# titu1994/tfdiffeq

Hardware: NVIDIA H100
Metric: accepted_rk_steps_x_state_elements_per_s (higher is better)
Workload: dtype f64

## Files before the change

### tfdiffeq_b200/csrc/b2ode_fused.cu

```cuda

#include "b2ode_dev.cuh"
#include "b2ode_rhs.cuh"
#include "b2ode_pay16.cuh"
#include <stdlib.h>
#include <mutex>

#ifdef B2ODE_FUSED_TRACE
constexpr int kTraceAttempts = 64, kTracePhases = 16;
__device__ unsigned long long g_fused_trace[2 * kTraceAttempts * kTracePhases];
#define FTRACE_DEP(att, ph, dep)                                                                                 \
    do {                                                                                                         \
        if ((unsigned)(dep) != 0x7ffffff3u && (threadIdx.x == 0 || threadIdx.x == blockDim.x - 32)  &&            \
            (blockIdx.x == 0 || blockIdx.x == gridDim.x - 1) && (att) >= 8 && (att) < 8 + kTraceAttempts)        \
            g_fused_trace[((blockIdx.x == 0 ? 0 : 1) * kTraceAttempts + ((att)-8)) * kTracePhases + (ph)] = clock64(); \
    } while (0)
#define FTRACE(att, ph) FTRACE_DEP(att, ph, 0)
extern "C" int b2ode_debug_fused_trace(unsigned long long *out) {
    B2_CUDA(cudaMemcpyFromSymbol(out, g_fused_trace, sizeof(g_fused_trace)));
    return 0;
}
#else
#define FTRACE(att, ph) do { } while (0)
#define FTRACE_DEP(att, ph, dep) do { } while (0)
#endif


struct FusedParams {
    b2ode_state *st;
    unsigned long long *part2;
    unsigned *ctr;
    const void *y0;
    void *out;
    unsigned *progress;
    int *host_mark;
    long long n_traj;
    int ncw;
    int have_first_step;
    double t_start, first_step;
    double time_sign;
    double rhs[8];
    const void *rhs_data;
    double beta[B2ODE_MAXK][B2ODE_MAXK];
    double c_sol[B2ODE_MAXK], c_error[B2ODE_MAXK], c_mid[B2ODE_MAXK];
    int fsal;
    double rtol0, atol0;
    CtrlParams c;
    CommParams comm;
};

__device__ __forceinline__ unsigned long long umax64(unsigned long long a, unsigned long long b) { return a > b ? a : b; }

template <int MODE>
__device__ __forceinline__ Pay pay_identity() {
    Pay r;
    r.a = 0.0;
    r.b = 0ull;
    r.flag = 0u;
    return r;
}

template <int MODE>
__device__ __forceinline__ Pay pay_combine(const Pay &x, const Pay &y) {
    Pay r;
    r.a = x.a + y.a;
    if (MODE == 0) r.b = x.b > y.b ? x.b : y.b;
    else r.b = (unsigned long long)__double_as_longlong(__longlong_as_double((long long)x.b) + __longlong_as_double((long long)y.b));
    r.flag = x.flag | y.flag;
    return r;
}

template <int MODE>
__device__ __forceinline__ Pay pay_warp_reduce(Pay x) {
#pragma unroll
    for (int o = 16; o > 0; o >>= 1) {
        Pay y;
        y.a = __shfl_xor_sync(0xffffffffu, x.a, o);
        y.b = __shfl_xor_sync(0xffffffffu, x.b, o);
        y.flag = __shfl_xor_sync(0xffffffffu, x.flag, o);
        x = pay_combine<MODE>(x, y);
    }
    return x;
}

__device__ __forceinline__ void pay_pack(const Pay &x, unsigned seq, unsigned long long (&w)[4]) {
    unsigned long long ab = (unsigned long long)__double_as_longlong(x.a);
    if (x.a != x.a) ab = 0x7ff8000000000000ull;
    ab = (ab & 0x7fffffffffffffffull) | ((unsigned long long)(x.flag & 1u) << 63);
    const unsigned long long s = (unsigned long long)seq << 32;
    w[0] = s | (ab & 0xffffffffull);
    w[1] = s | (ab >> 32);
    w[2] = s | (x.b & 0xffffffffull);
    w[3] = s | (x.b >> 32);
}

__device__ __forceinline__ Pay pay_unpack(const unsigned long long (&w)[4]) {
    const unsigned long long ab = (w[0] & 0xffffffffull) | (w[1] << 32);
    Pay r;
    r.flag = (unsigned)(ab >> 63);
    r.a = __longlong_as_double((long long)(ab & 0x7fffffffffffffffull));
    r.b = (w[2] & 0xffffffffull) | (w[3] << 32);
    return r;
}

template <bool SYS>
__device__ __forceinline__ void ll_store4(unsigned long long *dst, const unsigned long long (&w)[4]) {
    if (SYS) {
        asm volatile("st.relaxed.sys.global.v2.u64 [%0], {%1, %2};" ::"l"(dst), "l"(w[0]), "l"(w[1]) : "memory");
        asm volatile("st.relaxed.sys.global.v2.u64 [%0], {%1, %2};" ::"l"(dst + 2), "l"(w[2]), "l"(w[3]) : "memory");
    } else {
        asm volatile("st.relaxed.gpu.global.v2.u64 [%0], {%1, %2};" ::"l"(dst), "l"(w[0]), "l"(w[1]) : "memory");
        asm volatile("st.relaxed.gpu.global.v2.u64 [%0], {%1, %2};" ::"l"(dst + 2), "l"(w[2]), "l"(w[3]) : "memory");
    }
}

template <bool SYS>
__device__ __forceinline__ Pay ll_wait4(const unsigned long long *src, unsigned seq) {
    unsigned long long w[4];
    for (;;) {
        if (SYS) {
            asm volatile("ld.relaxed.sys.global.v2.u64 {%0, %1}, [%2];" : "=l"(w[0]), "=l"(w[1]) : "l"(src) : "memory");
            asm volatile("ld.relaxed.sys.global.v2.u64 {%0, %1}, [%2];" : "=l"(w[2]), "=l"(w[3]) : "l"(src + 2) : "memory");
        } else {
            asm volatile("ld.relaxed.gpu.global.v2.u64 {%0, %1}, [%2];" : "=l"(w[0]), "=l"(w[1]) : "l"(src) : "memory");
            asm volatile("ld.relaxed.gpu.global.v2.u64 {%0, %1}, [%2];" : "=l"(w[2]), "=l"(w[3]) : "l"(src + 2) : "memory");
        }
        if ((unsigned)(w[0] >> 32) == seq && (unsigned)(w[1] >> 32) == seq && (unsigned)(w[2] >> 32) == seq &&
            (unsigned)(w[3] >> 32) == seq)
            break;
    }
    return pay_unpack(w);
}

__device__ __forceinline__ void named_arrive(int id, int count) { asm volatile("bar.arrive %0, %1;" ::"r"(id), "r"(count) : "memory"); }
__device__ __forceinline__ void named_sync(int id, int count) { asm volatile("bar.sync %0, %1;" ::"r"(id), "r"(count) : "memory"); }

__device__ __forceinline__ unsigned long long opaque_zero() {
    unsigned long long c;
    asm volatile("mov.u64 %0, %%clock64;" : "=l"(c));
    return c >> 63;
}

constexpr int kGatherPerLane = 5;

struct FusedShared {
    Pay part[32];
    unsigned long long rlane[B2ODE_MAXPEERS][32][2];
    Pay tot;
    struct {
        double dt_next;
        int accept, done;
        unsigned status;
    } ctl;
};

constexpr int kBarPartials = 1, kBarDecision = 2, kBarRows = 3, kBarRowsReady = 4, kBarRemote = 5;

template <typename T, int S>
struct DenseConst {
    T cmid[S];
    T fc[5];
};

template <typename T>
__device__ __forceinline__ T fit_coef(int q) { return q == 0 ? T(-2) : q == 1 ? T(2) : q == 2 ? T(5) : q == 3 ? T(-3) : T(-4); }

template <typename T, int S>
__device__ __forceinline__ DenseConst<T, S> dense_const(const FusedParams &p, T dtc) {
    DenseConst<T, S> dc;
#pragma unroll
    for (int j = 0; j < S; ++j) dc.cmid[j] = Ar<T>::mul(dtc, (T)p.c_mid[j]);
#pragma unroll
    for (int q = 0; q < 5; ++q) dc.fc[q] = Ar<T>::mul(fit_coef<T>(q), dtc);
    return dc;
}

template <typename T, int S>
struct DenseShared {
    DenseConst<T, S> k;
    T x[3][4];
};

template <int MODE>
__device__ __forceinline__ void remote_gather(const FusedParams &p, FusedShared &sh, unsigned seq) {
    const int nranks = p.comm.nranks, lane = threadIdx.x & 31, rank = p.comm.rank;
#ifndef B2ODE_COMM_RG
#define B2ODE_COMM_RG 3
#endif
    constexpr int RG = B2ODE_COMM_RG;
    constexpr int NL = RG * kGatherPerLane;
    const unsigned long long *base = &p.comm.box[rank]->fused_part[seq & 1u][0][0][0] + (size_t)lane * 2;
    const unsigned tag = pay_tag(seq);
    for (int i0 = 0; i0 < nranks - 1; i0 += RG) {
        unsigned long long g0[NL], g1[NL];
        const unsigned long long *ptr[RG];
        unsigned mine = 0u;
#pragma unroll
        for (int r = 0; r < RG; ++r) {
            const int i = i0 + r;
            const bool ok = i < nranks - 1;
            const int src = ok ? (i < rank ? i : i + 1) : rank;
            const int G = ok ? p.comm.grid_of[src] : 0;
            ptr[r] = base + (size_t)src * (kMaxFusedBlocks * 2);
            asm volatile("" : "+l"(ptr[r]));
#pragma unroll
            for (int q = 0; q < kGatherPerLane; ++q)
                if (lane + 32 * q < G) mine |= 1u << (r * kGatherPerLane + q);
        }
        unsigned got;
        do {
            const unsigned long long z = opaque_zero();
#pragma unroll
            for (int r = 0; r < RG; ++r)
#pragma unroll
                for (int q = 0; q < kGatherPerLane; ++q)
                    asm volatile("ld.global.cg.v2.u64 {%0, %1}, [%2];"
                                 : "=l"(g0[r * kGatherPerLane + q]), "=l"(g1[r * kGatherPerLane + q])
                                 : "l"(ptr[r] + z + 64 * q)
                                 : "memory");
            got = 0u;
#pragma unroll
            for (int k = 0; k < NL; ++k) {
                got |= (pay_mismatch(g0[k], g1[k], tag) == 0u) ? (1u << k) : 0u;
            }
        } while ((got & mine) != mine);
#pragma unroll
        for (int r = 0; r < RG; ++r) {
            const int i = i0 + r;
            if (i >= nranks - 1) continue;
            const int src = i < rank ? i : i + 1;
            Pay acc = pay_identity<MODE>();
#pragma unroll
            for (int q = 0; q < kGatherPerLane; ++q)
                if ((mine >> (r * kGatherPerLane + q)) & 1u)
                    acc = pay_combine<MODE>(acc, pay_unpack16(g0[r * kGatherPerLane + q], g1[r * kGatherPerLane + q]));
            const int G = p.comm.grid_of[src];
            for (int b = lane + 32 * kGatherPerLane; b < G; b += 32) {
                const unsigned long long *sl = base + (size_t)src * (kMaxFusedBlocks * 2) + (size_t)(b - lane) * 2;
                unsigned long long a0, a1;
                do {
                    asm volatile("ld.global.cg.v2.u64 {%0, %1}, [%2];" : "=l"(a0), "=l"(a1) : "l"(sl + opaque_zero()) : "memory");
                } while (!pay_valid16(a0, a1, seq));
                acc = pay_combine<MODE>(acc, pay_unpack16(a0, a1));
            }
#ifdef B2ODE_COMM_RTOT
            acc = pay_warp_reduce<MODE>(acc);
#endif
            unsigned long long ab = (unsigned long long)__double_as_longlong(acc.a);
            if (acc.a != acc.a) ab = 0x7ff8000000000000ull;
            sh.rlane[src][lane][0] = (ab & 0x7fffffffffffffffull) | ((unsigned long long)(acc.flag & 1u) << 63);
            sh.rlane[src][lane][1] = acc.b;
        }
    }
    asm volatile("bar.arrive %0, %1;" ::"r"(kBarRemote), "r"(64) : "memory");
}

template <int MODE>
__device__ __forceinline__ Pay control_allreduce(const FusedParams &p, FusedShared &sh, int ncw, unsigned epoch, unsigned seq0,
                                                 unsigned long long hw2 = 0ull ,
                                                 int att = -1) {
    const int lane = threadIdx.x & 31;
    Pay x = (lane < ncw) ? sh.part[lane] : pay_identity<MODE>();
    x = pay_warp_reduce<MODE>(x);
    FTRACE_DEP(att, 2, __double_as_longlong(x.a));
    const int nranks = p.comm.nranks > 1 ? p.comm.nranks : 1, rank = p.comm.rank;
    const int G = (int)gridDim.x;
    const unsigned seq = seq0 + epoch, par = seq & 1u;
    unsigned long long w0, w1;
    pay_pack16(x, seq, w0, w1);
    if (nranks > 1 && epoch <= 2u && lane < nranks && lane != rank) {
        const int hw = (int)(par ? (unsigned)(hw2 >> 32) : (unsigned)hw2);
        for (int b = G + (int)blockIdx.x; b < hw && b < kMaxFusedBlocks; b += G) {
            unsigned long long *dst = &p.comm.box[lane]->fused_part[par][rank][b][0];
            asm volatile("st.relaxed.sys.global.v2.u64 [%0], {%1, %2};" ::"l"(dst), "l"(kPoisonW0), "l"(kPoisonW1) : "memory");
        }
    }
    if (nranks > 1 && lane < nranks && lane != rank) {
        unsigned long long *dst = &p.comm.box[lane]->fused_part[par][rank][blockIdx.x][0];
        asm volatile("st.relaxed.sys.global.v2.u64 [%0], {%1, %2};" ::"l"(dst), "l"(w0), "l"(w1) : "memory");
    }
    if (G > 1) {
        unsigned long long *slots = p.part2 + (size_t)par * G * 2;
        if (lane == 0) {
            asm volatile("st.relaxed.gpu.global.v2.u64 [%0], {%1, %2};" ::"l"(slots + (size_t)blockIdx.x * 2), "l"(w0), "l"(w1) : "memory");
            asm volatile("red.relaxed.gpu.global.add.u32 [%0], 1;" ::"l"(p.ctr) : "memory");
            const unsigned target = epoch * (unsigned)G;
            unsigned v;
            do {
                asm volatile("ld.relaxed.gpu.global.u32 %0, [%1];" : "=r"(v) : "l"(p.ctr) : "memory");
            } while ((int)(v - target) < 0);
        }
        __syncwarp();
        FTRACE(att, 3);
        unsigned long long g0[kGatherPerLane], g1[kGatherPerLane];
#pragma unroll
        for (int q = 0; q < kGatherPerLane; ++q) {
            const int b = lane + 32 * q;
            asm volatile("ld.global.cg.v2.u64 {%0, %1}, [%2];" : "=l"(g0[q]), "=l"(g1[q]) : "l"(slots + (size_t)(b < G ? b : 0) * 2) : "memory");
        }
        x = pay_identity<MODE>();
#pragma unroll
        for (int q = 0; q < kGatherPerLane; ++q) {
            const int b = lane + 32 * q;
            if (b < G) {
                while (!pay_valid16(g0[q], g1[q], seq))
                    asm volatile("ld.relaxed.gpu.global.v2.u64 {%0, %1}, [%2];" : "=l"(g0[q]), "=l"(g1[q]) : "l"(slots + (size_t)b * 2) : "memory");
                x = pay_combine<MODE>(x, pay_unpack16(g0[q], g1[q]));
            }
        }
        for (int b = lane + 32 * kGatherPerLane; b < G; b += 32) {
            unsigned long long a0, a1;
            do {
                asm volatile("ld.relaxed.gpu.global.v2.u64 {%0, %1}, [%2];" : "=l"(a0), "=l"(a1) : "l"(slots + (size_t)b * 2) : "memory");
            } while (!pay_valid16(a0, a1, seq));
            x = pay_combine<MODE>(x, pay_unpack16(a0, a1));
        }
    } else {
        x = (lane == 0) ? pay_unpack16(w0, w1) : pay_identity<MODE>();
    }
    if (nranks == 1) return pay_warp_reduce<MODE>(x);
#ifdef B2ODE_COMM_RTOT
    x = pay_warp_reduce<MODE>(x);
#endif
    asm volatile("bar.sync %0, %1;" ::"r"(kBarRemote), "r"(64) : "memory");
    Pay tot = pay_identity<MODE>();
    for (int q = 0; q < nranks; ++q) {
        Pay v = x;
        if (q != rank) {
            const unsigned long long a = sh.rlane[q][lane][0];
            v.flag = (unsigned)(a >> 63);
            v.a = __longlong_as_double((long long)(a & 0x7fffffffffffffffull));
            v.b = sh.rlane[q][lane][1];
        }
        tot = (q == 0) ? v : pay_combine<MODE>(tot, v);
    }
#ifdef B2ODE_COMM_RTOT
    return tot;
#else
    return pay_warp_reduce<MODE>(tot);
#endif
}

template <typename T>
__device__ __forceinline__ CtrlDecision ctrl_fast(const CtrlParams &c, double ssq, double mm, bool bad0, double dt) {
    const T tol = Ar<T>::add((T)c.atol[0], Ar<T>::mul((T)c.rtol[0], (T)mm));
    const double tol2n = (double)tol * (double)tol * (double)c.n_global[0];
    const double bound = std::is_same<T, float>::value ? tol2n * (1.0 + 5.9604644775390625e-08) : tol2n;
    CtrlDecision d;
    d.bad0 = bad0;
    d.accept = ssq <= bound;
    {
        const double lg = log2(((threadIdx.x & 31) == 0) ? ssq : tol2n);
        const double L = __shfl_sync(0xffffffffu, lg, 0) - __shfl_sync(0xffffffffu, lg, 1);
        const double df = (ssq < tol2n) ? 1.0 : c.dfactor;
        const double rf = c.safety * exp2(-0.5 * c.exponent * L);
        d.dt_next = (ssq == 0.0) ? dt * c.ifactor : dt * nan_min(c.ifactor, nan_max(df, rf));
    }
    d.m = 0.0;
    return d;
}


constexpr int fused_warps(int ntw, int tpt, int nsvc) { return (ntw + tpt - 1) / tpt + nsvc; }
constexpr int cmax(int a, int b) { return a > b ? a : b; }

template <typename T, typename RHS, int S, int MAXT>
struct FusedShape {
    static constexpr int tpt = (S == 7 && !(std::is_same<T, double>::value && RHS::D > 3)) ? 2 : 1;
    static constexpr int threads = 32 * cmax(fused_warps(MAXT / 32 - 1, tpt, 1), fused_warps(MAXT / 32 - 2, tpt, 2));
    static constexpr int min_blocks = tpt > 1 ? 1 : 0;
};

template <typename T, typename RHS, int S, int MAXT>
__global__ void __launch_bounds__(FusedShape<T, RHS, S, MAXT>::threads, FusedShape<T, RHS, S, MAXT>::min_blocks)
k_fused_adaptive(const __grid_constant__ FusedParams p) {
    constexpr int TPT = FusedShape<T, RHS, S, MAXT>::tpt;
    using A = Ar<T>;
    constexpr int D = RHS::D;
    constexpr int kMaxTraj = MAXT - 32;
    __shared__ FusedShared sh;
    __shared__ T sw[RHS::kSmem];
    __shared__ DenseShared<T, S> sdc;
    constexpr int kDenseRows = (3 * kMaxTraj * D * (int)sizeof(T) + (int)sizeof(FusedShared) + RHS::kSmem * (int)sizeof(T) +
                                (int)sizeof(DenseShared<T, S>) + 256 <= 48 * 1024) ? 3 : 2;
    __shared__ __align__(16) T s_rows[kDenseRows][kMaxTraj * D];
    const int nthreads = blockDim.x;
    const bool grouped = p.comm.nranks > 1;
    const int nsvc = grouped ? 2 : 1;
    const int pcw = (nthreads >> 5) - nsvc;
    const int ncw = p.ncw;
    const int nloc = 32 * (pcw + 1);
    const int warp = threadIdx.x >> 5, lane = threadIdx.x & 31;
    const bool is_control = warp == pcw;
    const unsigned ll_base = grouped ? (unsigned)p.comm.box[p.comm.rank]->ll_seq : 0u;
    const unsigned long long hw2 = (grouped && is_control) ? *(const volatile unsigned long long *)p.comm.box[p.comm.rank]->fused_hw : 0ull;
    if (RHS::kSmem > 1) {
        const int nw = (int)p.rhs[0] * 5 + 2;
        for (int q = threadIdx.x; q < nw && q < RHS::kSmem; q += nthreads) sw[q] = ((const T *)p.rhs_data)[q];
        __syncthreads();
    }
    const int n_out = p.c.n_out;
    const double *__restrict__ t_out = p.c.t_out;

    if (is_control) {
        unsigned epoch = 0;
        double t_cur = p.t_start, dt;
        unsigned status = 0;
        if (p.have_first_step) {
            dt = p.first_step;
        } else {
            named_sync(kBarPartials, nloc);
            Pay r = control_allreduce<1>(p, sh, ncw, ++epoch, ll_base, hw2);
            if (lane == 0) sh.tot = r;
            named_arrive(kBarDecision, nthreads);
            Partial tot;
            tot.v[0] = r.a;
            tot.v[1] = __longlong_as_double((long long)r.b);
            tot.v[2] = tot.v[3] = 0.0;
            T d1max;
            const T h0 = init_h0<T>(p.c, &tot, 1, &d1max);
            named_sync(kBarPartials, nloc);
            r = control_allreduce<1>(p, sh, ncw, ++epoch, ll_base, hw2);
            if (lane == 0) sh.tot = r;
            named_arrive(kBarDecision, nthreads);
            tot.v[0] = r.a;
            dt = (double)init_dt<T>(p.c, &tot, 1, h0, d1max);
        }
        int cur = 1;
        int done = (n_out <= 1) ? 1 : 0;
        if (!done && !(t_cur + dt > t_cur)) {
            status |= B2ODE_ST_UNDERFLOW;
            done = 1;
        }
        int late_rows = 0;
        double m_last = 0.0, t_prev = t_cur, dt_last = 0.0;
        unsigned long long n_acc = 0, n_rej = 0;
        long long nadv = 0;
        int att = 0;
        while (!done) {
            FTRACE(att, 0);
            const double t1_acc = t_cur + dt;
            int c2 = cur;
            while (c2 < n_out && __ldg(t_out + c2) <= t1_acc) ++c2;
            if (c2 > cur) {
                const T dtc = (T)dt, t0s = (T)t_cur, den = A::sub((T)t1_acc, t0s);
                if (lane < S) sdc.k.cmid[lane] = A::mul(dtc, (T)p.c_mid[lane]);
                if (lane < 5) sdc.k.fc[lane] = A::mul(fit_coef<T>(lane), dtc);
                if (lane < kDenseRows && cur + lane < c2) {
                    const T x = A::div(A::sub((T)__ldg(t_out + cur + lane), t0s), den);
                    const T x2 = A::mul(x, x), x3 = A::mul(x2, x), x4 = A::mul(x3, x);
                    sdc.x[lane][0] = x;
                    sdc.x[lane][1] = x2;
                    sdc.x[lane][2] = x3;
                    sdc.x[lane][3] = x4;
                }
                named_arrive(kBarRows, nloc);
            }
            named_sync(kBarPartials, nloc);
            if (late_rows) {
                __threadfence();
                if (lane == 0) {
                    const unsigned old = atomicAdd(p.progress, (unsigned)late_rows);
                    if (old + (unsigned)late_rows == (unsigned)(cur - 1) * gridDim.x) {
                        __threadfence_system();
                        *(volatile int *)p.host_mark = cur;
                    }
                }
                late_rows = 0;
            }
            FTRACE_DEP(att, 1, sh.part[0].flag);
            const Pay r = control_allreduce<0>(p, sh, ncw, ++epoch, ll_base, hw2, att);
            FTRACE_DEP(att, 4, __double_as_longlong(r.a));
            Partial tot;
            tot.v[0] = r.a;
            tot.v[1] = tot.v[2] = __longlong_as_double((long long)r.b);
            tot.v[3] = r.flag ? 1.0 : 0.0;
            CtrlDecision dec = ctrl_fast<T>(p.c, tot.v[0], tot.v[1], r.flag != 0u, dt);
            unsigned st_bits = status;
            if (dec.bad0) st_bits |= B2ODE_ST_NONFINITE;
            const bool adv = dec.accept && !dec.bad0;
            const double t1n = dec.accept ? t1_acc : t_cur;
            const int c_new = adv ? c2 : cur;
            const long long nadv2 = (c_new > cur) ? 0 : nadv + 1;
            int dn = (c_new >= n_out) ? 1 : 0;
            if (!dn) {
                if (nadv2 >= p.c.max_num_steps) st_bits |= B2ODE_ST_MAXSTEPS;
                if (!(t1n + dec.dt_next > t1n)) st_bits |= B2ODE_ST_UNDERFLOW;
            }
            if (st_bits) dn = 1;
            if (lane == 0) {
                sh.ctl.dt_next = dec.dt_next;
                sh.ctl.accept = dec.accept ? 1 : 0;
                sh.ctl.done = dn;
                sh.ctl.status = st_bits;
            }
            named_arrive(kBarDecision, nthreads);
            FTRACE_DEP(att, 5, __double_as_longlong(dec.dt_next));
            if (c2 > cur) named_sync(kBarRowsReady, nloc);
            if (adv && c2 > cur) {
                const long long first = (long long)blockIdx.x * (ncw * 32);
                long long nblk = p.n_traj - first;
                if (nblk > ncw * 32) nblk = ncw * 32;
                const int nel = (int)(nblk > 0 ? nblk * D : 0);
                const long long Nrow = p.n_traj * D;
                const int nrows = (c2 - cur) < kDenseRows ? (c2 - cur) : kDenseRows;
                for (int q = 0; q < nrows; ++q) {
                    T *row = (T *)p.out + (long long)(cur + q) * Nrow + first * D;
                    const T *src = s_rows[q];
                    constexpr int V = 16 / sizeof(T);
                    if ((reinterpret_cast<uintptr_t>(row) & 15u) == 0) {
                        const int nv = nel / V;
                        for (int e = lane; e < nv; e += 32)
                            reinterpret_cast<int4 *>(row)[e] = reinterpret_cast<const int4 *>(src)[e];
                        for (int e = nv * V + lane; e < nel; e += 32) row[e] = src[e];
                    } else {
                        for (int e = lane; e < nel; e += 32) row[e] = src[e];
                    }
                }
                if (p.host_mark) {
                    if (c2 - cur > kDenseRows) {
                        late_rows = c2 - cur;
                    } else {
                        __threadfence();
                        if (lane == 0) {
                            const unsigned old = atomicAdd(p.progress, (unsigned)(c2 - cur));
                            if (old + (unsigned)(c2 - cur) == (unsigned)(c2 - 1) * gridDim.x) {
                                __threadfence_system();
                                *(volatile int *)p.host_mark = c2;
                            }
                        }
                    }
                }
            }
            {
                const T tol = Ar<T>::add((T)p.c.atol[0], Ar<T>::mul((T)p.c.rtol[0], (T)tot.v[1]));
                dec.m = (double)(T)(tot.v[0] / ((double)tol * (double)tol * (double)p.c.n_global[0]));
            }
            m_last = dec.m;
            dt_last = dt;
            if (dec.accept) {
                n_acc += 1;
                t_prev = t_cur;
                t_cur = t1n;
            } else {
                n_rej += 1;
            }
            cur = c_new;
            nadv = nadv2;
            dt = dec.dt_next;
            status = st_bits;
            done = dn;
            ++att;
        }
        if (blockIdx.x == 0 && lane == 0) {
            b2ode_state z;
            memset(&z, 0, sizeof(z));
            z.t0 = t_prev;
            z.t1 = t_cur;
            z.dt = dt;
            z.dt_last = dt_last;
            z.msr_max = m_last;
            z.n_acc = n_acc;
            z.n_rej = n_rej;
            z.attempt = n_acc + n_rej;
            z.n_steps_adv = nadv;
            z.done = 1;
            z.status = status;
            z.cursor = cur;
            z.xseq = p.st->xseq;
            *p.st = z;
        }
        if (blockIdx.x == 0 && grouped) {
            if (lane == 0) {
                Mailbox *mb = p.comm.box[p.comm.rank];
                mb->ll_seq = (unsigned long long)(ll_base + epoch);
                if (epoch >= 1u) mb->fused_hw[(ll_base + 1u) & 1u] = gridDim.x;
                if (epoch >= 2u) mb->fused_hw[(ll_base + 2u) & 1u] = gridDim.x;
            }
        }
        return;
    }

    if (warp == pcw + 1) {
        unsigned epoch = 0;
        double t_cur = p.t_start, dt;
        if (p.have_first_step) {
            dt = p.first_step;
        } else {
            remote_gather<1>(p, sh, ll_base + (++epoch));
            named_sync(kBarDecision, nthreads);
            Partial tot;
            tot.v[0] = sh.tot.a;
            tot.v[1] = __longlong_as_double((long long)sh.tot.b);
            tot.v[2] = tot.v[3] = 0.0;
            T d1max;
            const T h0 = init_h0<T>(p.c, &tot, 1, &d1max);
            remote_gather<1>(p, sh, ll_base + (++epoch));
            named_sync(kBarDecision, nthreads);
            tot.v[0] = sh.tot.a;
            dt = (double)init_dt<T>(p.c, &tot, 1, h0, d1max);
        }
        int done = (n_out <= 1) ? 1 : 0;
        if (!done && !(t_cur + dt > t_cur)) done = 1;
        while (!done) {
            remote_gather<0>(p, sh, ll_base + (++epoch));
            named_sync(kBarDecision, nthreads);
            done = sh.ctl.done;
        }
        return;
    }

    long long i[TPT];
    int vw[TPT];
    bool live[TPT];
#pragma unroll
    for (int u = 0; u < TPT; ++u) {
        vw[u] = warp + u * pcw;
        i[u] = (long long)blockIdx.x * (ncw * 32) + vw[u] * 32 + lane;
        live[u] = vw[u] < ncw && i[u] < p.n_traj;
    }
    const long long N = p.n_traj * D;
    const T *y0g = (const T *)p.y0;
    T *out = (T *)p.out;
    const T tsign = (T)p.time_sign;
    T y[TPT][D], f0[TPT][D];
#pragma unroll
    for (int u = 0; u < TPT; ++u) {
#pragma unroll
        for (int d = 0; d < D; ++d) y[u][d] = live[u] ? y0g[i[u] * D + d] : T(0);
        if (live[u]) {
#pragma unroll
            for (int d = 0; d < D; ++d) out[i[u] * D + d] = y[u][d];
        }
    }
    auto rhs = [&](T t, const T(&yy)[D], T(&dy)[D]) {
        if (tsign < T(0)) {
            RHS::eval(p.rhs, sw, -t, yy, dy);
#pragma unroll
            for (int d = 0; d < D; ++d) dy[d] = -dy[d];
        } else {
            RHS::eval(p.rhs, sw, t, yy, dy);
        }
    };
    auto contribute = [&](const auto &mine, auto mode) {
        constexpr int MODE = decltype(mode)::value;
        Pay w[TPT];
#pragma unroll
        for (int u = 0; u < TPT; ++u) w[u] = pay_warp_reduce<MODE>(mine[u]);
        if (lane == 0) {
#pragma unroll
            for (int u = 0; u < TPT; ++u)
                if (vw[u] < ncw) sh.part[vw[u]] = w[u];
        }
        named_arrive(kBarPartials, nloc);
    };
    double t_cur = p.t_start;
#pragma unroll
    for (int u = 0; u < TPT; ++u) rhs((T)t_cur, y[u], f0[u]);

    double dt;
    if (p.have_first_step) {
        dt = p.first_step;
    } else {
        const T rtol = (T)p.rtol0, atol = (T)p.atol0;
        T scale[TPT][D];
        Pay mine[TPT];
#pragma unroll
        for (int u = 0; u < TPT; ++u) {
            mine[u] = pay_identity<1>();
            double s0 = 0.0, s1 = 0.0;
#pragma unroll
            for (int d = 0; d < D; ++d) {
                scale[u][d] = A::add(atol, A::mul(A::abs(y[u][d]), rtol));
                if (live[u]) {
                    const double q0 = (double)A::div(y[u][d], scale[u][d]), q1 = (double)A::div(f0[u][d], scale[u][d]);
                    s0 += q0 * q0;
                    s1 += q1 * q1;
                }
            }
            mine[u].a = s0;
            mine[u].b = (unsigned long long)__double_as_longlong(s1);
        }
        contribute(mine, IC<1>{});
        named_sync(kBarDecision, nthreads);
        Partial tot;
        tot.v[0] = sh.tot.a;
        tot.v[1] = __longlong_as_double((long long)sh.tot.b);
        tot.v[2] = tot.v[3] = 0.0;
        T d1max;
        const T h0 = init_h0<T>(p.c, &tot, 1, &d1max);
#pragma unroll
        for (int u = 0; u < TPT; ++u) {
            T y1[D], f1[D];
#pragma unroll
            for (int d = 0; d < D; ++d) y1[d] = A::add(y[u][d], A::mul(h0, f0[u][d]));
            rhs(A::add((T)t_cur, h0), y1, f1);
            double s2 = 0.0;
            if (live[u]) {
#pragma unroll
                for (int d = 0; d < D; ++d) {
                    const double q = (double)A::div(A::sub(f1[d], f0[u][d]), scale[u][d]);
                    s2 += q * q;
                }
            }
            mine[u].a = s2;
            mine[u].b = 0ull;
        }
        contribute(mine, IC<1>{});
        named_sync(kBarDecision, nthreads);
        tot.v[0] = sh.tot.a;
        dt = (double)init_dt<T>(p.c, &tot, 1, h0, d1max);
    }
    int cur = 1;
    int done = (n_out <= 1) ? 1 : 0;
    if (!done && !(t_cur + dt > t_cur)) done = 1;

    int att = 0;
    while (!done) {
        const T t0c = (T)t_cur, dtc = (T)dt;
        T k[S][TPT][D];
#pragma unroll
        for (int u = 0; u < TPT; ++u)
#pragma unroll
            for (int d = 0; d < D; ++d) k[0][u][d] = f0[u][d];
        T yi[TPT][D];
#pragma unroll
        for (int s = 0; s < S - 1; ++s) {
            const T ti = A::add(t0c, A::mul((T)p.c.alpha[s], dtc));
            T acc[TPT][D];
#pragma unroll
            for (int j = 0; j <= s; ++j) {
                const T c = A::mul(dtc, (T)p.beta[s][j]);
#pragma unroll
                for (int u = 0; u < TPT; ++u)
#pragma unroll
                    for (int d = 0; d < D; ++d) {
                        const T term = A::mul(c, k[j][u][d]);
                        acc[u][d] = (j == 0) ? term : A::add(acc[u][d], term);
                    }
            }
#pragma unroll
            for (int u = 0; u < TPT; ++u) {
#pragma unroll
                for (int d = 0; d < D; ++d) yi[u][d] = A::add(y[u][d], acc[u][d]);
                rhs(ti, yi[u], k[s + 1][u]);
            }
        }
        if (!p.fsal) {
            T acc[TPT][D];
#pragma unroll
            for (int j = 0; j < S; ++j) {
                const T c = A::mul(dtc, (T)p.c_sol[j]);
#pragma unroll
                for (int u = 0; u < TPT; ++u)
#pragma unroll
                    for (int d = 0; d < D; ++d) {
                        const T term = A::mul(c, k[j][u][d]);
                        acc[u][d] = (j == 0) ? term : A::add(acc[u][d], term);
                    }
            }
#pragma unroll
            for (int u = 0; u < TPT; ++u)
#pragma unroll
                for (int d = 0; d < D; ++d) yi[u][d] = A::add(y[u][d], acc[u][d]);
        }
        {
            Pay mine[TPT];
            T err[TPT][D];
#pragma unroll
            for (int j = 0; j < S; ++j) {
                const T c = A::mul(dtc, (T)p.c_error[j]);
#pragma unroll
                for (int u = 0; u < TPT; ++u)
#pragma unroll
                    for (int d = 0; d < D; ++d) {
                        const T term = A::mul(c, k[j][u][d]);
                        err[u][d] = (j == 0) ? term : A::add(err[u][d], term);
                    }
            }
#pragma unroll
            for (int u = 0; u < TPT; ++u) {
                mine[u] = pay_identity<0>();
                if (live[u]) {
                    double sum = 0.0;
                    unsigned long long m0 = 0ull, m1 = 0ull;
#pragma unroll
                    for (int d = 0; d < D; ++d) {
                        const double ed = (double)err[u][d];
                        sum += ed * ed;
                        m0 = umax64(m0, (unsigned long long)__double_as_longlong(fabs((double)y[u][d])));
                        m1 = umax64(m1, (unsigned long long)__double_as_longlong(fabs((double)yi[u][d])));
                    }
                    mine[u].a = sum;
                    mine[u].b = umax64(m0, m1);
                    mine[u].flag = (m0 >= 0x7ff0000000000000ull) ? 1u : 0u;
                }
            }
            contribute(mine, IC<0>{});
        }
        FTRACE(att, 8);
        const double t1_acc = t_cur + dt;
        int c2 = cur;
        while (c2 < n_out && __ldg(t_out + c2) <= t1_acc) ++c2;
        const T t0s = t0c, t1s = (T)t1_acc;
        auto fit = [&](int u, const DenseConst<T, S> &dc, T(&ca)[D], T(&cb)[D], T(&cc)[D], T(&cd)[D]) {
            T ymid[D];
            {
                T acc[D];
#pragma unroll
                for (int j = 0; j < S; ++j) {
                    const T c = dc.cmid[j];
#pragma unroll
                    for (int d = 0; d < D; ++d) {
                        const T term = A::mul(c, k[j][u][d]);
                        acc[d] = (j == 0) ? term : A::add(acc[d], term);
                    }
                }
#pragma unroll
                for (int d = 0; d < D; ++d) ymid[d] = A::add(y[u][d], acc[d]);
            }
#pragma unroll
            for (int d = 0; d < D; ++d) {
                const T f0e = k[0][u][d], f1e = k[S - 1][u][d], y0e = y[u][d], y1e = yi[u][d];
                T a = A::mul(dc.fc[0], f0e);
                a = A::add(a, A::mul(dc.fc[1], f1e));
                a = A::add(a, A::mul(T(-8), y0e));
                a = A::add(a, A::mul(T(-8), y1e));
                a = A::add(a, A::mul(T(16), ymid[d]));
                T b = A::mul(dc.fc[2], f0e);
                b = A::add(b, A::mul(dc.fc[3], f1e));
                b = A::add(b, A::mul(T(18), y0e));
                b = A::add(b, A::mul(T(14), y1e));
                b = A::add(b, A::mul(T(-32), ymid[d]));
                T cq = A::mul(dc.fc[4], f0e);
                cq = A::add(cq, A::mul(dtc, f1e));
                cq = A::add(cq, A::mul(T(-11), y0e));
                cq = A::add(cq, A::mul(T(-5), y1e));
                cq = A::add(cq, A::mul(T(16), ymid[d]));
                ca[d] = a;
                cb[d] = b;
                cc[d] = cq;
                cd[d] = A::mul(dtc, f0e);
            }
        };
        auto eval_x = [&](int u, T x, T x2, T x3, T x4, const T(&ca)[D], const T(&cb)[D], const T(&cc)[D], const T(&cd)[D],
                          T(&r)[D]) {
#pragma unroll
            for (int d = 0; d < D; ++d) {
                T v = A::mul(ca[d], x4);
                v = A::add(v, A::mul(cb[d], x3));
                v = A::add(v, A::mul(cc[d], x2));
                v = A::add(v, A::mul(cd[d], x));
                r[d] = A::add(v, y[u][d]);
            }
        };
        const bool blk_out = c2 > cur;
        if (blk_out) {
            named_sync(kBarRows, nloc);
#pragma unroll
            for (int u = 0; u < TPT; ++u) {
                if (live[u]) {
                    T ca[D], cb[D], cc[D], cd[D];
                    fit(u, sdc.k, ca, cb, cc, cd);
#pragma unroll
                    for (int q = 0; q < kDenseRows; ++q) {
                        if (cur + q < c2) {
                            T r[D];
                            eval_x(u, sdc.x[q][0], sdc.x[q][1], sdc.x[q][2], sdc.x[q][3], ca, cb, cc, cd, r);
#pragma unroll
                            for (int d = 0; d < D; ++d) s_rows[q][(vw[u] * 32 + lane) * D + d] = r[d];
                        }
                    }
                }
            }
        }
        if (blk_out) named_arrive(kBarRowsReady, nloc);
        FTRACE(att, 9);
        named_sync(kBarDecision, nthreads);
        const bool accept = sh.ctl.accept != 0;
        FTRACE_DEP(att, 10, sh.ctl.accept);
        if (accept) {
            if (blk_out && cur + kDenseRows < c2) {
                const DenseConst<T, S> dc = dense_const<T, S>(p, dtc);
                const T den = A::sub(t1s, t0s);
#pragma unroll
                for (int u = 0; u < TPT; ++u) {
                    if (!live[u]) continue;
                    T ca[D], cb[D], cc[D], cd[D];
                    fit(u, dc, ca, cb, cc, cd);
                    for (int j = cur + kDenseRows; j < c2; ++j) {
                        const T x = A::div(A::sub((T)__ldg(t_out + j), t0s), den);
                        const T x2 = A::mul(x, x), x3 = A::mul(x2, x), x4 = A::mul(x3, x);
                        T r[D];
                        eval_x(u, x, x2, x3, x4, ca, cb, cc, cd, r);
                        T *row = out + (long long)j * N + i[u] * D;
#pragma unroll
                        for (int d = 0; d < D; ++d) row[d] = r[d];
                    }
                }
            }
            t_cur = t1_acc;
            cur = c2;
#pragma unroll
            for (int u = 0; u < TPT; ++u)
#pragma unroll
                for (int d = 0; d < D; ++d) {
                    y[u][d] = yi[u][d];
                    f0[u][d] = k[S - 1][u][d];
                }
        }
        dt = sh.ctl.dt_next;
        done = sh.ctl.done;
        ++att;
    }
}

struct FusedDevInfo {
    bool ready;
    int coop, nsm;
    int per_sm[33];
};
constexpr int kFusedMaxDevices = 64;

template <typename T, typename RHS, int S, int MAXT>
static int fused_dev_info(const FusedDevInfo **out) {
    static std::mutex mu;
    static FusedDevInfo info[kFusedMaxDevices];
    int dev = 0;
    B2_CUDA(cudaGetDevice(&dev));
    if (dev < 0 || dev >= kFusedMaxDevices) return b2_fail(B2ODE_EINVAL, "device ordinal %d out of range", dev);
    std::lock_guard<std::mutex> lock(mu);
    FusedDevInfo &d = info[dev];
    if (!d.ready) {
        B2_CUDA(cudaDeviceGetAttribute(&d.coop, cudaDevAttrCooperativeLaunch, dev));
        B2_CUDA(cudaDeviceGetAttribute(&d.nsm, cudaDevAttrMultiProcessorCount, dev));
        for (int w = 2; w <= FusedShape<T, RHS, S, MAXT>::threads / 32; ++w)
            B2_CUDA(cudaOccupancyMaxActiveBlocksPerMultiprocessor(&d.per_sm[w], k_fused_adaptive<T, RHS, S, MAXT>, 32 * w, 0));
        d.ready = true;
    }
    *out = &d;
    return 0;
}

template <int MAXT, int TPT>
static int fused_geometry(const FusedDevInfo &di, long long n_traj, int nsvc, int *ncw_out, int *grid_out) {
    const int nsm = di.nsm;
    const int kMaxNcw = MAXT / 32 - nsvc;
    long long per_block = (n_traj + nsm - 1) / nsm;
    int ncw = (int)((per_block + 31) / 32);
    if (ncw < 1) ncw = 1;
    if (ncw > kMaxNcw) ncw = kMaxNcw;
    for (; ncw >= 1; --ncw) {
        const int grid = (int)((n_traj + (long long)ncw * 32 - 1) / ((long long)ncw * 32));
        if (grid <= di.per_sm[fused_warps(ncw, TPT, nsvc)] * nsm) {
            *ncw_out = ncw;
            *grid_out = grid;
            return 0;
        }
    }
    return b2_fail(B2ODE_ENOMEM, "batch of %lld trajectories cannot stay co-resident on %d SMs", n_traj, nsm);
}

template <typename T, typename RHS, int S, int MAXT>
static int fused_launch(const FusedParams &p_in, long long n_traj, cudaStream_t st, long long *capacity, const int64_t *n_traj_rank) {
    constexpr int TPT = FusedShape<T, RHS, S, MAXT>::tpt;
    const FusedDevInfo *di = nullptr;
    {
        const int rc = fused_dev_info<T, RHS, S, MAXT>(&di);
        if (rc) return rc;
    }
    if (capacity) {
        long long best = 0;
        for (int ncw = MAXT / 32 - 2; ncw >= 1 && di->coop; --ncw) {
            const long long cap = (long long)di->per_sm[fused_warps(ncw, TPT, 2)] * di->nsm * ncw * 32;
            if (cap > best) best = cap;
        }
        *capacity = best;
        return 0;
    }
    if (!di->coop) return b2_fail(B2ODE_ESTATE, "device does not support cooperative launch");
    FusedParams p = p_in;
    const int nsvc = p.comm.nranks > 1 ? 2 : 1;
    int ncw = 0, grid = 0;
    {
        const int rc = fused_geometry<MAXT, TPT>(*di, n_traj, nsvc, &ncw, &grid);
        if (rc) return rc;
    }
    if (p.comm.nranks > 1) {
        for (int r = 0; r < p.comm.nranks; ++r) {
            int ncw_r = 0, grid_r = 0;
            const int rc = fused_geometry<MAXT, TPT>(*di, n_traj_rank[r], nsvc, &ncw_r, &grid_r);
            if (rc) return rc;
            if (grid_r > kMaxFusedBlocks)
                return b2_fail(B2ODE_ENOMEM, "rank %d needs %d blocks, the group mailbox holds %d", r, grid_r, kMaxFusedBlocks);
            p.comm.grid_of[r] = grid_r;
        }
        if (p.comm.grid_of[p.comm.rank] != grid) return b2_fail(B2ODE_ESTATE, "inconsistent shard size for this rank");
    }
    p.ncw = ncw;
    void *args[] = {(void *)&p};
    const int slot = b2_timing_begin(6 , st);
    B2_CUDA(cudaLaunchCooperativeKernel((const void *)k_fused_adaptive<T, RHS, S, MAXT>, dim3(grid),
                                        dim3(32 * fused_warps(ncw, TPT, nsvc)), args, 0, st));
    b2_timing_end(6, slot, st);
    b2_count_launch();
    return 0;
}

template <typename T, typename RHS>
static int fused_dispatch_s(const FusedParams &p, int n_k, long long n_traj, cudaStream_t st, long long *capacity,
                            const int64_t *ntr) {
    switch (n_k) {
        case 2: return fused_launch<T, RHS, 2, 512>(p, n_traj, st, capacity, ntr);
        case 4: return fused_launch<T, RHS, 4, 512>(p, n_traj, st, capacity, ntr);
        case 7: return fused_launch<T, RHS, 7, 576>(p, n_traj, st, capacity, ntr);
        case 14: return fused_launch<T, RHS, 14, 256>(p, n_traj, st, capacity, ntr);
    }
    return b2_fail(B2ODE_EINVAL, "fused solve supports tableaus with 2, 4, 7 or 14 k's (got %d)", n_k);
}

template <typename T>
static int fused_dispatch_rhs(const FusedParams &p, int rhs_kind, int n_k, long long n_traj, cudaStream_t st,
                              long long *capacity = nullptr, const int64_t *ntr = nullptr) {
    switch (rhs_kind) {
        case B2ODE_RHS_LORENZ: return fused_dispatch_s<T, RhsLorenz<T>>(p, n_k, n_traj, st, capacity, ntr);
        case B2ODE_RHS_LOTKA_VOLTERRA: return fused_dispatch_s<T, RhsLotkaVolterra<T>>(p, n_k, n_traj, st, capacity, ntr);
        case B2ODE_RHS_CUBIC_MLP: return fused_dispatch_s<T, RhsCubicMLP<T>>(p, n_k, n_traj, st, capacity, ntr);
        case B2ODE_RHS_KEPLER: return fused_dispatch_s<T, RhsKepler<T>>(p, n_k, n_traj, st, capacity, ntr);
    }
    return b2_fail(B2ODE_EINVAL, "unknown built-in right-hand side %d", rhs_kind);
}

extern "C" int64_t b2ode_fused_capacity(const b2ode_adaptive_desc *desc, int rhs_kind) {
    if (!desc) return b2_fail(B2ODE_EINVAL, "null argument");
    FusedParams p;
    memset(&p, 0, sizeof(p));
    long long cap = 0;
    int rc;
    if (desc->dtype == B2ODE_F64) rc = fused_dispatch_rhs<double>(p, rhs_kind, desc->n_k, 0, nullptr, &cap);
    else if (desc->dtype == B2ODE_F32) rc = fused_dispatch_rhs<float>(p, rhs_kind, desc->n_k, 0, nullptr, &cap);
    else return b2_fail(B2ODE_EINVAL, "dtype must be 0 or 1");
    if (rc) return rc < 0 ? rc : -rc;
    return (int64_t)cap;
}

static int rhs_dim(int kind) {
    return kind == B2ODE_RHS_LORENZ ? 3 : (kind == B2ODE_RHS_LOTKA_VOLTERRA || kind == B2ODE_RHS_CUBIC_MLP) ? 2 : kind == B2ODE_RHS_KEPLER ? 4 : -1;
}

static int rhs_check(int kind, const double *prm, int n_prm, const void *rhs_data) {
    if (kind == B2ODE_RHS_CUBIC_MLP) {
        if (n_prm < 2 || !rhs_data) return b2_fail(B2ODE_EINVAL, "cubic-MLP right-hand side needs {H, cube} and its weights");
        if (prm[0] < 1 || prm[0] > 128) return b2_fail(B2ODE_EINVAL, "cubic-MLP hidden width must be in [1, 128]");
    }
    return 0;
}

extern "C" size_t b2ode_fused_workspace_bytes(int64_t n_traj) {
    const long long grid_max = (n_traj + 31) / 32;
    return (size_t)256 + (size_t)grid_max * 32;
}

extern "C" int b2ode_fused_solve(const b2ode_adaptive_desc *desc, const b2ode_fused_desc *f) {
    if (!desc || !f) return b2_fail(B2ODE_EINVAL, "null argument");
    if (!f->y0 || !f->out || !f->t_out || !f->state || !f->workspace) return b2_fail(B2ODE_EINVAL, "null buffer");
    const int rhs_kind = f->rhs_kind;
    const int D = rhs_dim(rhs_kind);
    if (D < 0) return b2_fail(B2ODE_EINVAL, "unknown built-in right-hand side %d", rhs_kind);
    if (desc->nseg != 1 || desc->seg_len[0] % D != 0) return b2_fail(B2ODE_EINVAL, "state must be one (B, %d) tensor", D);
    if (desc->dense_kind != 0) return b2_fail(B2ODE_EINVAL, "fused solve supports the quartic dense output only");
    if (f->n_rhs_params < 0 || f->n_rhs_params > 8) return b2_fail(B2ODE_EINVAL, "bad rhs params");
    const long long n_traj = desc->seg_len[0] / D;
    if (n_traj < 1) return b2_fail(B2ODE_EINVAL, "empty batch");
    if (f->workspace_bytes < b2ode_fused_workspace_bytes(n_traj)) return b2_fail(B2ODE_ENOMEM, "workspace too small");
    cudaStream_t st = (cudaStream_t)f->cuda_stream;
    unsigned char *w = (unsigned char *)f->workspace;
    if ((uintptr_t)w & 15u) return b2_fail(B2ODE_EINVAL, "workspace must be 16-byte aligned");
    const int nranks = f->nranks > 1 ? f->nranks : 1;
    FusedParams p;
    memset(&p, 0, sizeof(p));
    B2_CUDA(cudaMemsetAsync(w, 0, 256, st));
    p.progress = (unsigned *)(w + 128);
    p.host_mark = (int *)f->host_mark;
    p.st = (b2ode_state *)f->state;
    p.y0 = f->y0;
    p.out = f->out;
    p.n_traj = n_traj;
    p.have_first_step = (f->first_step == f->first_step) ? 1 : 0;
    p.t_start = f->t_start;
    p.first_step = f->first_step;
    p.time_sign = f->time_sign;
    for (int i = 0; i < f->n_rhs_params; ++i) p.rhs[i] = f->rhs_params[i];
    p.rhs_data = f->rhs_data;
    {
        const int rc_ = rhs_check(rhs_kind, f->rhs_params, f->n_rhs_params, f->rhs_data);
        if (rc_) return rc_;
    }
    const int nk = desc->n_k;
    for (int i = 0; i < B2ODE_MAXK; ++i) {
        for (int j = 0; j < B2ODE_MAXK; ++j) p.beta[i][j] = desc->beta[i][j];
        p.c_sol[i] = desc->c_sol[i];
        p.c_error[i] = desc->c_error[i];
        p.c_mid[i] = desc->c_mid[i];
        p.c.alpha[i] = desc->alpha[i];
    }
    p.fsal = desc->fsal;
    p.rtol0 = desc->rtol[0];
    p.atol0 = desc->atol[0];
    p.c.n_k = nk;
    p.c.controller = desc->controller;
    p.c.rtol[0] = desc->rtol[0];
    p.c.atol[0] = desc->atol[0];
    p.c.safety = desc->safety;
    p.c.ifactor = desc->ifactor;
    p.c.dfactor = desc->dfactor;
    p.c.exponent = desc->exponent;
    p.c.inv_safety = 1.0 / desc->safety;
    p.c.inv_ifactor = 1.0 / desc->ifactor;
    p.c.inv_dfactor = 1.0 / desc->dfactor;
    p.c.max_num_steps = desc->max_num_steps;
    p.c.init_order = desc->init_order;
    p.c.n_out = f->n_out;
    p.c.t_out = f->t_out;
    p.c.tstage = nullptr;
    long long n_glob = n_traj;
    p.comm.rank = 0;
    p.comm.nranks = 0;
    if (nranks > 1) {
        if (!f->mailboxes || nranks > B2ODE_MAXPEERS || f->rank < 0 || f->rank >= nranks) return b2_fail(B2ODE_EINVAL, "bad group arguments");
        n_glob = 0;
        for (int r = 0; r < nranks; ++r) {
            if (!f->mailboxes[r] || f->n_traj_rank[r] < 1) return b2_fail(B2ODE_EINVAL, "bad mailbox / shard size of rank %d", r);
            n_glob += f->n_traj_rank[r];
            p.comm.box[r] = (Mailbox *)f->mailboxes[r];
        }
        if (f->n_traj_rank[f->rank] != n_traj) return b2_fail(B2ODE_EINVAL, "n_traj_rank[rank] does not match the state");
        p.comm.rank = f->rank;
        p.comm.nranks = nranks;
    }
    B2_CUDA(cudaMemsetAsync(w + 256, 0, b2ode_fused_workspace_bytes(n_traj) - 256, st));
    p.ctr = (unsigned *)w;
    p.part2 = (unsigned long long *)(w + 256);
    p.c.n_global[0] = n_glob * D;
    if (desc->dtype == B2ODE_F64) return fused_dispatch_rhs<double>(p, rhs_kind, nk, n_traj, st, nullptr, f->n_traj_rank);
    if (desc->dtype == B2ODE_F32) return fused_dispatch_rhs<float>(p, rhs_kind, nk, n_traj, st, nullptr, f->n_traj_rank);
    return b2_fail(B2ODE_EINVAL, "dtype must be 0 or 1");
}

struct FusedFixedParams {
    const void *y0;
    void *out;
    long long n_traj;
    int n_steps, n_out, method;
    const void *times;
    const void *dts;
    const int *j0;
    const unsigned char *ends;
    const void *s1;
    const void *s2;
    double time_sign;
    double rhs[8];
    const void *rhs_data;
};

template <typename T, typename RHS>
__global__ void __launch_bounds__(256) k_fused_fixed(const __grid_constant__ FusedFixedParams p) {
    using A = Ar<T>;
    constexpr int D = RHS::D;
    __shared__ T sw[RHS::kSmem];
    if (RHS::kSmem > 1) {
        const int nw = (int)p.rhs[0] * 5 + 2;
        for (int q = threadIdx.x; q < nw && q < RHS::kSmem; q += 256) sw[q] = ((const T *)p.rhs_data)[q];
        __syncthreads();
    }
    const T tsign = (T)p.time_sign;
    auto rhs = [&](T t, const T(&yy)[D], T(&dy)[D]) {
        if (tsign < T(0)) {
            RHS::eval(p.rhs, sw, -t, yy, dy);
#pragma unroll
            for (int d = 0; d < D; ++d) dy[d] = -dy[d];
        } else {
            RHS::eval(p.rhs, sw, t, yy, dy);
        }
    };
    const long long N = p.n_traj * D;
    const T *times = (const T *)p.times, *dts = (const T *)p.dts, *s1 = (const T *)p.s1, *s2 = (const T *)p.s2;
// ... 111 lines not shown
```

Measured before the change: 32.61 billion.

## Precompute dt-scaled tableau coefficients in shared memory and fold time sign into dt

```diff
diff --git a/tfdiffeq_b200/csrc/b2ode_fused.cu b/tfdiffeq_b200/csrc/b2ode_fused.cu
--- a/tfdiffeq_b200/csrc/b2ode_fused.cu
+++ b/tfdiffeq_b200/csrc/b2ode_fused.cu
@@ -134,6 +134,17 @@
 __device__ __forceinline__ void named_arrive(int id, int count) { asm volatile("bar.arrive %0, %1;" ::"r"(id), "r"(count) : "memory"); }
 __device__ __forceinline__ void named_sync(int id, int count) { asm volatile("bar.sync %0, %1;" ::"r"(id), "r"(count) : "memory"); }
 
+__device__ __forceinline__ int ntid_fresh() {
+    int v;
+    asm volatile("mov.u32 %0, %%ntid.x;" : "=r"(v));
+    return v;
+}
+
+__device__ __forceinline__ double negate_if(double x, bool neg) {
+    return __longlong_as_double(__double_as_longlong(x) ^ (neg ? (long long)0x8000000000000000ull : 0ll));
+}
+__device__ __forceinline__ float negate_if(float x, bool neg) { return __int_as_float(__float_as_int(x) ^ (neg ? (int)0x80000000u : 0)); }
+
 __device__ __forceinline__ unsigned long long opaque_zero() {
     unsigned long long c;
     asm volatile("mov.u64 %0, %%clock64;" : "=l"(c));
@@ -153,7 +164,7 @@
     } ctl;
 };
 
-constexpr int kBarPartials = 1, kBarDecision = 2, kBarRows = 3, kBarRowsReady = 4, kBarRemote = 5;
+constexpr int kBarPartials = 1, kBarDecision = 2, kBarRows = 3, kBarRowsReady = 4, kBarRemote = 5, kBarFirstStep = 6;
 
 template <typename T, int S>
 struct DenseConst {
@@ -179,6 +190,25 @@
     DenseConst<T, S> k;
     T x[3][4];
 };
+
+template <typename T, int S>
+struct StageConst {
+    static constexpr int nb = S * (S - 1) / 2, n = nb + 2 * S;
+    static constexpr __host__ __device__ int beta(int s, int j) { return s * (s + 1) / 2 + j; }
+    static constexpr __host__ __device__ int err(int j) { return nb + j; }
+    static constexpr __host__ __device__ int sol(int j) { return nb + S + j; }
+    __align__(16) T c[n];
+};
+
+template <typename T, int S>
+__device__ __forceinline__ T stage_coef(const FusedParams &p, int idx) {
+    using SC = StageConst<T, S>;
+    if (idx >= SC::sol(0)) return (T)p.c_sol[idx - SC::sol(0)];
+    if (idx >= SC::err(0)) return (T)p.c_error[idx - SC::err(0)];
+    int s = 0;
+    while (idx > s) idx -= ++s;
+    return (T)p.beta[s][idx];
+}
 
 template <int MODE>
 __device__ __forceinline__ void remote_gather(const FusedParams &p, FusedShared &sh, unsigned seq) {
@@ -380,8 +410,9 @@
     __shared__ FusedShared sh;
     __shared__ T sw[RHS::kSmem];
     __shared__ DenseShared<T, S> sdc;
+    __shared__ StageConst<T, S> ssc;
     constexpr int kDenseRows = (3 * kMaxTraj * D * (int)sizeof(T) + (int)sizeof(FusedShared) + RHS::kSmem * (int)sizeof(T) +
-                                (int)sizeof(DenseShared<T, S>) + 256 <= 48 * 1024) ? 3 : 2;
+                                (int)sizeof(DenseShared<T, S>) + (int)sizeof(StageConst<T, S>) + 256 <= 48 * 1024) ? 3 : 2;
     __shared__ __align__(16) T s_rows[kDenseRows][kMaxTraj * D];
     const int nthreads = blockDim.x;
     const bool grouped = p.comm.nranks > 1;
@@ -425,6 +456,19 @@
             tot.v[0] = r.a;
             dt = (double)init_dt<T>(p.c, &tot, 1, h0, d1max);
         }
+        constexpr int kSc = StageConst<T, S>::n, kScLane = (kSc + 31) / 32;
+        T scoef[kScLane];
+#pragma unroll
+        for (int q = 0; q < kScLane; ++q) scoef[q] = (lane + 32 * q < kSc) ? stage_coef<T, S>(p, lane + 32 * q) : T(0);
+        const bool rev = (T)p.time_sign < T(0);
+        auto publish_stage = [&](double dtn) {
+            const T dtk = negate_if((T)dtn, rev);
+#pragma unroll
+            for (int q = 0; q < kScLane; ++q)
+                if (lane + 32 * q < kSc) ssc.c[lane + 32 * q] = A::mul(dtk, scoef[q]);
+        };
+        publish_stage(dt);
+        named_arrive(kBarFirstStep, nloc);
         int cur = 1;
         int done = (n_out <= 1) ? 1 : 0;
         if (!done && !(t_cur + dt > t_cur)) {
@@ -442,9 +486,9 @@
             int c2 = cur;
             while (c2 < n_out && __ldg(t_out + c2) <= t1_acc) ++c2;
             if (c2 > cur) {
-                const T dtc = (T)dt, t0s = (T)t_cur, den = A::sub((T)t1_acc, t0s);
-                if (lane < S) sdc.k.cmid[lane] = A::mul(dtc, (T)p.c_mid[lane]);
-                if (lane < 5) sdc.k.fc[lane] = A::mul(fit_coef<T>(lane), dtc);
+                const T dtk = negate_if((T)dt, rev), t0s = (T)t_cur, den = A::sub((T)t1_acc, t0s);
+                if (lane < S) sdc.k.cmid[lane] = A::mul(dtk, (T)p.c_mid[lane]);
+                if (lane < 5) sdc.k.fc[lane] = A::mul(fit_coef<T>(lane), dtk);
                 if (lane < kDenseRows && cur + lane < c2) {
                     const T x = A::div(A::sub((T)__ldg(t_out + cur + lane), t0s), den);
                     const T x2 = A::mul(x, x), x3 = A::mul(x2, x), x4 = A::mul(x3, x);
@@ -487,6 +531,7 @@
                 if (!(t1n + dec.dt_next > t1n)) st_bits |= B2ODE_ST_UNDERFLOW;
             }
             if (st_bits) dn = 1;
+            publish_stage(dec.dt_next);
             if (lane == 0) {
                 sh.ctl.dt_next = dec.dt_next;
                 sh.ctl.accept = dec.accept ? 1 : 0;
@@ -621,7 +666,7 @@
     const long long N = p.n_traj * D;
     const T *y0g = (const T *)p.y0;
     T *out = (T *)p.out;
-    const T tsign = (T)p.time_sign;
+    const bool rev = (T)p.time_sign < T(0);
     T y[TPT][D], f0[TPT][D];
 #pragma unroll
     for (int u = 0; u < TPT; ++u) {
@@ -632,26 +677,23 @@
             for (int d = 0; d < D; ++d) out[i[u] * D + d] = y[u][d];
         }
     }
-    auto rhs = [&](T t, const T(&yy)[D], T(&dy)[D]) {
-        if (tsign < T(0)) {
-            RHS::eval(p.rhs, sw, -t, yy, dy);
-#pragma unroll
-            for (int d = 0; d < D; ++d) dy[d] = -dy[d];
-        } else {
-            RHS::eval(p.rhs, sw, t, yy, dy);
-        }
-    };
+    auto rhs = [&](T t, const T(&yy)[D], T(&dy)[D]) { RHS::eval(p.rhs, sw, rev ? -t : t, yy, dy); };
+    auto bar_all = [&]() { return S <= 7 ? ntid_fresh() : nthreads; };
+    auto bar_loc = [&]() { return S <= 7 ? ntid_fresh() - (p.comm.nranks > 1 ? 32 : 0) : nloc; };
     auto contribute = [&](const auto &mine, auto mode) {
         constexpr int MODE = decltype(mode)::value;
         Pay w[TPT];
 #pragma unroll
         for (int u = 0; u < TPT; ++u) w[u] = pay_warp_reduce<MODE>(mine[u]);
         if (lane == 0) {
-#pragma unroll
-            for (int u = 0; u < TPT; ++u)
-                if (vw[u] < ncw) sh.part[vw[u]] = w[u];
-        }
-        named_arrive(kBarPartials, nloc);
+            const int pcw_f = TPT > 1 ? (ntid_fresh() >> 5) - (p.comm.nranks > 1 ? 2 : 1) : pcw;
+#pragma unroll
+            for (int u = 0; u < TPT; ++u) {
+                const int v = warp + u * pcw_f;
+                if (v < ncw) sh.part[v] = w[u];
+            }
+        }
+        named_arrive(kBarPartials, bar_loc());
     };
     double t_cur = p.t_start;
 #pragma unroll
@@ -687,12 +729,12 @@
         tot.v[1] = __longlong_as_double((long long)sh.tot.b);
         tot.v[2] = tot.v[3] = 0.0;
         T d1max;
-        const T h0 = init_h0<T>(p.c, &tot, 1, &d1max);
+        const T h0 = init_h0<T>(p.c, &tot, 1, &d1max), hk = negate_if(h0, rev);
 #pragma unroll
         for (int u = 0; u < TPT; ++u) {
             T y1[D], f1[D];
 #pragma unroll
-            for (int d = 0; d < D; ++d) y1[d] = A::add(y[u][d], A::mul(h0, f0[u][d]));
+            for (int d = 0; d < D; ++d) y1[d] = A::add(y[u][d], A::mul(hk, f0[u][d]));
             rhs(A::add((T)t_cur, h0), y1, f1);
             double s2 = 0.0;
             if (live[u]) {
@@ -713,10 +755,13 @@
     int cur = 1;
     int done = (n_out <= 1) ? 1 : 0;
     if (!done && !(t_cur + dt > t_cur)) done = 1;
-
+    named_sync(kBarFirstStep, nloc);
+
+    using SC = StageConst<T, S>;
     int att = 0;
     while (!done) {
         const T t0c = (T)t_cur, dtc = (T)dt;
+        const T dtk = negate_if(dtc, rev);
         T k[S][TPT][D];
 #pragma unroll
         for (int u = 0; u < TPT; ++u)
@@ -729,7 +774,7 @@
             T acc[TPT][D];
 #pragma unroll
             for (int j = 0; j <= s; ++j) {
-                const T c = A::mul(dtc, (T)p.beta[s][j]);
+                const T c = ssc.c[SC::beta(s, j)];
 #pragma unroll
                 for (int u = 0; u < TPT; ++u)
 #pragma unroll
@@ -749,7 +794,7 @@
             T acc[TPT][D];
 #pragma unroll
             for (int j = 0; j < S; ++j) {
-                const T c = A::mul(dtc, (T)p.c_sol[j]);
+                const T c = ssc.c[SC::sol(j)];
 #pragma unroll
                 for (int u = 0; u < TPT; ++u)
 #pragma unroll
@@ -768,7 +813,7 @@
             T err[TPT][D];
 #pragma unroll
             for (int j = 0; j < S; ++j) {
-                const T c = A::mul(dtc, (T)p.c_error[j]);
+                const T c = ssc.c[SC::err(j)];
 #pragma unroll
                 for (int u = 0; u < TPT; ++u)
 #pragma unroll
@@ -832,14 +877,14 @@
                 b = A::add(b, A::mul(T(14), y1e));
                 b = A::add(b, A::mul(T(-32), ymid[d]));
                 T cq = A::mul(dc.fc[4], f0e);
-                cq = A::add(cq, A::mul(dtc, f1e));
+                cq = A::add(cq, A::mul(dtk, f1e));
                 cq = A::add(cq, A::mul(T(-11), y0e));
                 cq = A::add(cq, A::mul(T(-5), y1e));
                 cq = A::add(cq, A::mul(T(16), ymid[d]));
                 ca[d] = a;
                 cb[d] = b;
                 cc[d] = cq;
-                cd[d] = A::mul(dtc, f0e);
+                cd[d] = A::mul(dtk, f0e);
             }
         };
         auto eval_x = [&](int u, T x, T x2, T x3, T x4, const T(&ca)[D], const T(&cb)[D], const T(&cc)[D], const T(&cd)[D],
@@ -855,7 +900,7 @@
         };
         const bool blk_out = c2 > cur;
         if (blk_out) {
-            named_sync(kBarRows, nloc);
+            named_sync(kBarRows, bar_loc());
 #pragma unroll
             for (int u = 0; u < TPT; ++u) {
                 if (live[u]) {
@@ -873,14 +918,14 @@
                 }
             }
         }
-        if (blk_out) named_arrive(kBarRowsReady, nloc);
+        if (blk_out) named_arrive(kBarRowsReady, bar_loc());
         FTRACE(att, 9);
-        named_sync(kBarDecision, nthreads);
+        named_sync(kBarDecision, bar_all());
         const bool accept = sh.ctl.accept != 0;
         FTRACE_DEP(att, 10, sh.ctl.accept);
         if (accept) {
             if (blk_out && cur + kDenseRows < c2) {
-                const DenseConst<T, S> dc = dense_const<T, S>(p, dtc);
+                const DenseConst<T, S> dc = dense_const<T, S>(p, dtk);
                 const T den = A::sub(t1s, t0s);
 #pragma unroll
                 for (int u = 0; u < TPT; ++u) {
```

Measured after the change: 38.33 billion (median of 6 runs). +17.6%, better.
